# mmeidlinger/lut_ldpc

Measured on AMD Instinct MI355X. Metric: decoded codewords/sec, DVB-S2 N=64800 4-bit LUT 50-iter, higher is better.
Workload: dtype u8

## Files before the change

### lut_ldpc_amd/csrc/hip/decoder_frontend.hip

```cpp
#include "decoder_state.hpp"
#include "kernels_frontend.hpp"
#include "kernels_encode.hpp"

#pragma GCC visibility push(hidden)

hipError_t preload_frontend_kernels() {
    hipFuncAttributes a;
    return hipFuncGetAttributes(&a, reinterpret_cast<const void *>(&encode_random_kernel));
}

static int fill_cells(const lutldpc_channel_cells *c, const lutldpc_decoder *d, ChannelCells &C) {
    if (!c || !c->thr || !c->cha_label || !c->msg_label || !c->slicer_neg || !c->cha_label_mirror || !c->msg_label_mirror)
        return fail(LUTLDPC_ERR_ARG, "channel cells: NULL member");
    if (c->n_cells < 1 || c->n_cells > kMaxCells) return fail(LUTLDPC_ERR_ARG, "channel cells: n_cells outside [1,72]");
    std::memset(&C, 0, sizeof(C));
    C.n_cells = c->n_cells;
    for (int j = 0; j < c->n_cells; j++) {
        if (j < c->n_cells - 1) { C.thr[j] = c->thr[j]; if (j && c->thr[j] < c->thr[j - 1]) return fail(LUTLDPC_ERR_ARG, "channel cells: thresholds must ascend"); }
        if (c->cha_label[j] >= d->Nq_Cha || c->cha_label_mirror[j] >= d->Nq_Cha || c->msg_label[j] >= d->Nq_Msg[0] || c->msg_label_mirror[j] >= d->Nq_Msg[0])
            return fail(LUTLDPC_ERR_ARG, "channel cells: label outside its alphabet");
        C.cha[j] = c->cha_label[j]; C.msg[j] = c->msg_label[j]; C.neg[j] = c->slicer_neg[j] ? 1 : 0;
        C.cha_m[j] = c->cha_label_mirror[j]; C.msg_m[j] = c->msg_label_mirror[j];
    }
    return LUTLDPC_OK;
// ... 8 lines not shown
    HIP_TRY(hipMemsetAsync(d->d_stats.p, 0, sizeof(int32_t) * (size_t)Bpad * 4, d->stream));
    const uint8_t *cw = nullptr;
    if (codewords_host) {
        HIP_TRY(d->d_codewords.alloc((size_t)B * N));
        HIP_TRY(hipMemcpyAsync(d->d_codewords.p, codewords_host, (size_t)B * N, hipMemcpyHostToDevice, d->stream));
        cw = d->d_codewords.p;
    }
    Timed t(d, LUTLDPC_K_FRONTEND);
    const int ppt = 8, npairs = (N + 1) / 2;
    dim3 grid((unsigned)((npairs + 4 * ppt - 1) / (4 * ppt)), (unsigned)G);
    DEV_PARAM(dC, d, C);
    if (sent_rows)
        PACK_DISPATCH(d, launch_k(sample_labels_kernel<PK, true>, grid, dim3(256), 0, d->stream, dC, (uint32_t)seed, (uint32_t)(seed >> 32), stream, frame0, B, N,
                           sent_rows, d->d_cha_t.p, d->d_msg0_t.p, d->d_stats.p, ppt));
    else
        PACK_DISPATCH(d, launch_k(sample_labels_kernel<PK>, grid, dim3(256), 0, d->stream, dC, (uint32_t)seed, (uint32_t)(seed >> 32), stream, frame0, B, N, cw,
                           d->d_cha_t.p, d->d_msg0_t.p, d->d_stats.p, ppt));
    LAUNCH_CHECK();
    return LUTLDPC_OK;
}

static int encode_tiles(lutldpc_decoder *d, uint64_t seed, uint32_t stream, uint64_t frame0, int B) {
    if (!d->gen_set) return fail(LUTLDPC_ERR_STATE, "no generator set: random codewords on the device need lutldpc_decoder_set_generator first");
    const int Bpad = d->bpad(B), G = Bpad / d->tile(), N = d->nvar;
    const int RB = d->pack == 2 ? sent_row_bytes<2>() : sent_row_bytes<1>();
    HIP_TRY(d->d_sent.alloc((size_t)G * N * RB));
    Timed t(d, LUTLDPC_K_FRONTEND);
    const int K = d->gen_K, R = d->gen_R;
    const int W128 = (K + 127) / 128, T = (R + kEncTileRows - 1) / kEncTileRows, W32 = (K + 31) / 32;
    const unsigned gx = (unsigned)(Bpad / kEncFrames), gy = (unsigned)std::max(1, (std::max(T, (W32 + 7) / 8) + 3) / 4);
    launch_k(encode_random_kernel, dim3(gx, gy), dim3(256), (size_t)W128 * kEncFrames * 16, d->stream, d->d_gen.p, K, R, d->gen_W32p,
             (uint32_t)seed, (uint32_t)(seed >> 32), stream, frame0, B, N, d->tile(), d->d_sent.p);
    LAUNCH_CHECK();
    return LUTLDPC_OK;
}

static int launch_sent_to_bytes(lutldpc_decoder *d, uint8_t *dst, int B) {
    const size_t n = (size_t)B * d->nvar;
    PACK_DISPATCH(d, launch_k(sent_rows_to_bytes_kernel<PK>, dim3((unsigned)((n + 255) / 256)), dim3(256), 0, d->stream, d->d_sent.p, B, d->nvar, dst));
    LAUNCH_CHECK();
    return LUTLDPC_OK;
}

static int sim_batch_impl(lutldpc_decoder *d, const lutldpc_channel_cells *cells, uint64_t seed, uint32_t stream, uint64_t frame0, int B,
                   const uint8_t *codewords, bool device_codewords, int K_info, int32_t *frame_stats, uint8_t *cha_out, uint8_t *bits_out) {
    if (!d || !frame_stats) return fail(LUTLDPC_ERR_ARG, "NULL argument");
    if (d->device < 0) return fail(LUTLDPC_ERR_STATE, "decoder was created without a device (host-only handle)");
    if (B <= 0 || K_info < 0 || K_info > d->nvar) return fail(LUTLDPC_ERR_ARG, "bad B / K_info");
    if (device_codewords && !d->gen_set) return fail(LUTLDPC_ERR_STATE, "sim_batch_random: no generator set (lutldpc_decoder_set_generator)");
    ChannelCells C;
    int rc = fill_cells(cells, d, C);
    if (rc) return rc;
    HIP_TRY(hipSetDevice(d->device));
    if (device_codewords) {
        if ((rc = ensure_batch(d, B))) return rc;
        if ((rc = encode_tiles(d, seed, stream, frame0, B))) return rc;
    }
    if ((rc = sample_tiles(d, C, seed, stream, frame0, B, codewords, device_codewords ? d->d_sent.p : nullptr))) return rc;
    if ((rc = decode_tiles(d, B))) return rc;
    {
        Timed t(d, LUTLDPC_K_FRONTEND);
        const int Bpad = d->bpad(B), G = Bpad / d->tile(), rpw = 64;
        const int rows = K_info > 0 ? K_info : 1;
        const dim3 grid((unsigned)((rows + 4 * rpw - 1) / (4 * rpw)), (unsigned)G);
        if (device_codewords)
            PACK_DISPATCH(d, launch_k(count_errors_kernel<PK, true>, grid, dim3(256), 0, d->stream, d->d_hard.p, d->d_sent.p, B, d->nvar, K_info, d->d_iters.p,
                               d->d_stats.p, rpw));
        else
            PACK_DISPATCH(d, launch_k(count_errors_kernel<PK>, grid, dim3(256), 0, d->stream, d->d_hard.p,
                               codewords ? d->d_codewords.p : nullptr, B, d->nvar, K_info, d->d_iters.p, d->d_stats.p, rpw));
        LAUNCH_CHECK();
    }
    HIP_TRY(hipMemcpyAsync(frame_stats, d->d_stats.p, sizeof(int32_t) * (size_t)B * 4, hipMemcpyDeviceToHost, d->stream));
    if (cha_out || bits_out) {
        const int Bpad = d->bpad(B), G = Bpad / d->tile(), N = d->nvar;
        const size_t n = (size_t)B * N;
        HIP_TRY(d->d_out_bits.alloc(n));
        if (cha_out) {
            if ((rc = launch_transpose_out(d, d->d_cha_t.p, d->d_out_bits.p, B, G))) return rc;
            LAUNCH_CHECK();
            HIP_TRY(hipMemcpyAsync(cha_out, d->d_out_bits.p, n, hipMemcpyDeviceToHost, d->stream));
        }
        if (bits_out) {
            if ((rc = launch_transpose_out(d, d->d_hard.p, d->d_out_bits.p, B, G))) return rc;
            LAUNCH_CHECK();
            HIP_TRY(hipMemcpyAsync(bits_out, d->d_out_bits.p, n, hipMemcpyDeviceToHost, d->stream));
        }
    }
    HIP_TRY(hipStreamSynchronize(d->stream));
    return LUTLDPC_OK;
}

#pragma GCC visibility pop

extern "C" {

int lutldpc_decoder_sim_batch(lutldpc_decoder *d, const lutldpc_channel_cells *cells, uint64_t seed, uint32_t stream, uint64_t frame0, int B,
                              const uint8_t *codewords, int K_info, int32_t *frame_stats, uint8_t *cha_out, uint8_t *bits_out) {
    return sim_batch_impl(d, cells, seed, stream, frame0, B, codewords, false, K_info, frame_stats, cha_out, bits_out);
}

int lutldpc_decoder_sim_batch_random(lutldpc_decoder *d, const lutldpc_channel_cells *cells, uint64_t seed, uint32_t stream, uint64_t frame0, int B,
                                     int K_info, int32_t *frame_stats, uint8_t *cha_out, uint8_t *bits_out) {
    return sim_batch_impl(d, cells, seed, stream, frame0, B, nullptr, true, K_info, frame_stats, cha_out, bits_out);
}

int lutldpc_decoder_set_generator(lutldpc_decoder *d, int K, int R, const uint64_t *rows) {
    if (!d) return fail(LUTLDPC_ERR_ARG, "NULL decoder");
    if (!rows) return fail(LUTLDPC_ERR_ARG, "generator rows are NULL");
    if (K < 1 || R < 0 || K + R != d->nvar) return fail(LUTLDPC_ERR_ARG, "generator: K + R must equal nvar (K >= 1)");
    if (d->device < 0) return fail(LUTLDPC_ERR_STATE, "decoder was created without a device (host-only handle)");
    if (K > kEncMaxInfoBits) return fail(LUTLDPC_ERR_UNSUPPORTED, "generator: more than 8192 information bits (device encoder limit)");
    HIP_TRY(hipSetDevice(d->device));
    const int WK = (K + 63) / 64, W32p = 4 * ((K + 127) / 128), Rp = (R + kEncTileRows - 1) / kEncTileRows * kEncTileRows;
    std::vector<uint32_t> a((size_t)std::max(Rp, 1) * W32p, 0u);
    for (int i = 0; i < R; i++)
        for (int j = 0; j < 2 * WK; j++) {
            const int k0 = 32 * j;
            uint32_t w = (uint32_t)(rows[(size_t)i * WK + (size_t)(j >> 1)] >> (32 * (j & 1)));
            if (k0 + 32 > K) w &= k0 >= K ? 0u : (1u << (K - k0)) - 1u;
            a[(size_t)i * W32p + (size_t)j] = w;
        }
    HIP_TRY(hipStreamSynchronize(d->stream));
    HIP_TRY(d->d_gen.upload(a));
    d->gen_K = K; d->gen_R = R; d->gen_W32p = W32p; d->gen_set = true;
    make_describe(d);
    return LUTLDPC_OK;
}

int lutldpc_decoder_encode_random(lutldpc_decoder *d, uint64_t seed, uint32_t stream, uint64_t frame0, int B, uint8_t *codewords) {
    if (!d) return fail(LUTLDPC_ERR_ARG, "NULL decoder");
    if (B <= 0) return fail(LUTLDPC_ERR_ARG, "B must be positive");
    if (d->device < 0) return fail(LUTLDPC_ERR_STATE, "decoder was created without a device (host-only handle)");
    HIP_TRY(hipSetDevice(d->device));
    int rc = encode_tiles(d, seed, stream, frame0, B);
    if (rc) return rc;
    if (codewords) {
        const size_t n = (size_t)B * d->nvar;
        HIP_TRY(d->d_out_bits.alloc(n));
        if ((rc = launch_sent_to_bytes(d, d->d_out_bits.p, B))) return rc;
        HIP_TRY(hipMemcpyAsync(codewords, d->d_out_bits.p, n, hipMemcpyDeviceToHost, d->stream));
    }
    HIP_TRY(hipStreamSynchronize(d->stream));
    return LUTLDPC_OK;
}

int lutldpc_decoder_sample_labels(lutldpc_decoder *d, const lutldpc_channel_cells *cells, uint64_t seed, uint32_t stream, uint64_t frame0, int B,
                                  const uint8_t *codewords, uint8_t *cha, uint8_t *msg0) {
    if (!d || !cha || !msg0) return fail(LUTLDPC_ERR_ARG, "NULL argument");
    if (d->device < 0) return fail(LUTLDPC_ERR_STATE, "decoder was created without a device (host-only handle)");
    if (B <= 0) return fail(LUTLDPC_ERR_ARG, "B must be positive");
    ChannelCells C;
    int rc = fill_cells(cells, d, C);
    if (rc) return rc;
    HIP_TRY(hipSetDevice(d->device));
    if ((rc = sample_tiles(d, C, seed, stream, frame0, B, codewords))) return rc;
    const int Bpad = d->bpad(B), G = Bpad / d->tile(), N = d->nvar;
    const size_t n = (size_t)B * N;
    HIP_TRY(d->d_in_cha.alloc(n)); HIP_TRY(d->d_in_msg.alloc(n));
    if ((rc = launch_transpose_out(d, d->d_cha_t.p, d->d_in_cha.p, B, G))) return rc;
    if ((rc = launch_transpose_out(d, d->d_msg0_t.p, d->d_in_msg.p, B, G))) return rc;
    HIP_TRY(hipMemcpyAsync(cha, d->d_in_cha.p, n, hipMemcpyDeviceToHost, d->stream));
    HIP_TRY(hipMemcpyAsync(msg0, d->d_in_msg.p, n, hipMemcpyDeviceToHost, d->stream));
    HIP_TRY(hipStreamSynchronize(d->stream));
    return LUTLDPC_OK;
}

// ... 2 lines not shown
```

### lut_ldpc_amd/csrc/hip/decoder_state.hpp

```cpp
#pragma once
#include "../../../include/lut_ldpc_hip.h"
#include "kernels_common.hpp"
#include "kernels_fast.hpp"
#include "lut_program.hpp"
#include "jit.hpp"
#include "jit_resident.hpp"

#include <algorithm>
#include <array>
#include <cmath>
#include <cstdio>
#include <cstring>
#include <map>
#include <memory>
#include <mutex>
#include <sstream>
#include <string>
#include <vector>

namespace lutldpc { LUTLDPC_FAST_LAUNCHERS(extern) }

using namespace lutldpc;

#pragma GCC visibility push(hidden)
// ... 159 lines not shown
    std::vector<std::vector<const JitKernel *>> var_jit, dec_jit, chk_jit;
    std::string jit_log;
    struct GraphSlot { int seen = 0; hipGraphExec_t exec = nullptr; };
    std::map<std::array<int, 4>, GraphSlot> graphs;
    void drop_graphs() { for (auto &kv : graphs) if (kv.second.exec) (void)hipGraphExecDestroy(kv.second.exec); graphs.clear(); }
    int cn_epw() const { return opt.cn_edges_per_wave > 0 ? opt.cn_edges_per_wave : 42; }
    int npw_vn(int deg) const { return opt.nodes_per_wave > 0 ? opt.nodes_per_wave : std::max(1, opt.vn_edges_per_wave / std::max(deg, 1)); }
    int npw_cn(int deg) const { return opt.nodes_per_wave_cn > 0 ? opt.nodes_per_wave_cn : std::max(1, cn_epw() / std::max(deg, 1)); }
    int npw_cn_class(size_t ci) const { return ci < cn_npw_class.size() && cn_npw_class[ci] > 0 ? cn_npw_class[ci] : npw_cn(cclass[ci].deg); }
    std::string place_info = "null";
    struct SkewSlot { int n_roles = 0; size_t role_off = 0; const int32_t *items = nullptr; int nb = 0; int state_half = -1, state_ii = 0; };
    struct SkewPlan { std::vector<SkewSlot> slots; std::vector<RoleParams> h_roles; DevBuf<RoleParams> d_roles; };
    std::map<std::array<int, 3>, std::unique_ptr<SkewPlan>> skew_plans;
    std::map<std::pair<std::vector<int>, std::vector<int>>, DevBuf<int32_t>> item_tabs;
    void drop_plans() { skew_plans.clear(); item_tabs.clear(); }
    int tile() const { return kRowBytes * pack; }
    int bpad(int B) const { return (B + tile() - 1) / tile() * tile(); }
    bool profiling = false;
    struct Ev { hipEvent_t a, b; int kind; };
    std::vector<Ev> ev_live;
    std::vector<hipEvent_t> ev_pool;
    double prof_ms[LUTLDPC_K_COUNT] = {0};
    int64_t prof_n[LUTLDPC_K_COUNT] = {0};
    std::string describe;

    lutldpc_decoder() = default;
    lutldpc_decoder(const lutldpc_decoder &) = delete;
    lutldpc_decoder &operator=(const lutldpc_decoder &) = delete;
    ~lutldpc_decoder();
};

#pragma GCC visibility push(hidden)

#define LAUNCH_CHECK()                                                                              \
    do {                                                                                            \
        hipError_t e_ = hipGetLastError();                                                          \
        if (e_ != hipSuccess) return fail(LUTLDPC_ERR_HIP, std::string("kernel launch: ") + hipGetErrorString(e_)); \
        if (d->opt.validate) {                                                                      \
            e_ = hipStreamSynchronize(d->stream);                                                   \
            if (e_ == hipSuccess) e_ = hipGetLastError();                                           \
            if (e_ != hipSuccess) return fail(LUTLDPC_ERR_HIP, std::string("launch failed on the device (") + __func__ + ":" + std::to_string(__LINE__) + "): " + hipGetErrorString(e_)); \
        }                                                                                           \
    } while (0)

const void *dev_param_bytes(lutldpc_decoder *d, const void *src, size_t n);
template <class T> const T *dev_param(lutldpc_decoder *d, const T &v) { return static_cast<const T *>(dev_param_bytes(d, &v, sizeof(T))); }
#define DEV_PARAM(var, d, v)                      \
    const auto *var = dev_param((d), (v));        \
    if (!var) return LUTLDPC_ERR_HIP

#define PACK_DISPATCH(d, ...)                        \
    do {                                             \
        if ((d)->pack == 2) { constexpr int PK = 2; __VA_ARGS__; } \
        else { constexpr int PK = 1; __VA_ARGS__; }  \
    } while (0)

hipEvent_t ev_get(lutldpc_decoder *d);
void prof_fold(lutldpc_decoder *d);
struct Timed {
    lutldpc_decoder *d; int kind; hipEvent_t a{}, b{};
    Timed(lutldpc_decoder *d_, int k) : d(d_), kind(k) {
        if (d->profiling) { a = ev_get(d); b = ev_get(d); (void)hipEventRecord(a, d->stream); }
    }
    ~Timed() {
        if (d->profiling) { (void)hipEventRecord(b, d->stream); d->ev_live.push_back({a, b, kind}); }
    }
};
void make_describe(lutldpc_decoder *d);

void build_classes(const std::vector<int> &deg, std::vector<NodeClass> &cls, std::vector<int> &list);
int compile_all(lutldpc_decoder *d);
int upload_static(lutldpc_decoder *d);
struct JitRegistry { std::mutex mu; std::map<std::string, JitKernel> by_src; };
constexpr size_t kJitRegistryMax = 4096;
JitRegistry &jit_registry();
JitKernel *jit_get(int device, const std::string &src, std::string &log);
bool jit_class_source(const lutldpc_decoder *d, int kind, size_t s, size_t i, std::string &src, std::string &err);

int ensure_batch(lutldpc_decoder *d, int B);
int check_batch_buffers(const lutldpc_decoder *d, int Bpad);

hipError_t preload_stream_kernels();
int launch_state(lutldpc_decoder *d, int B, int Bpad, int mode, int value, int f0 = 0, int f1 = -1, int sel = 0);
int launch_transpose_out(lutldpc_decoder *d, const uint8_t *src_rows, uint8_t *dst, int B, int G, int rows = 0);
int launch_quantize_llr(lutldpc_decoder *d, size_t n, int n_qb_Cha, int n_qb_Msg, int mode);
bool chain_active(const lutldpc_decoder *d, int set);
bool late_hard_active(const lutldpc_decoder *d, bool skewed, bool *chain_skip);
int launch_late_hard(lutldpc_decoder *d, bool skewed, int g0, int G, const int32_t *ctl);
int decode_tiles(lutldpc_decoder *d, int B);
int decode_device(lutldpc_decoder *d, const uint8_t *d_cha, const uint8_t *d_msg0, int B, uint8_t *d_out_bits, int32_t *d_out_iters);

struct HalfRange { int g0, G; };
hipError_t preload_compact_kernels();
bool skew_eligible(const lutldpc_decoder *d);
bool compaction_on(const lutldpc_decoder *d, int G);
int compaction_min_groups(const lutldpc_decoder *d);
int launch_uncompaction(lutldpc_decoder *d, const HalfRange (&half)[2], int Bpad);
int iterate_skewed(lutldpc_decoder *d, int B, int Bpad, int G);

ResidentSpec resident_spec(const lutldpc_decoder *d, int S, int NT);
bool resident_eligible(const lutldpc_decoder *d);
bool resident_pick(const lutldpc_decoder *d, int G, int &S_out, int &NT_out, int &lds_out);
inline bool resident_active(const lutldpc_decoder *d) { return d->resident_ok && d->opt.use_resident; }
int resident_plan_for(lutldpc_decoder *d, int G, lutldpc_decoder::ResidentPlan **out);
int launch_resident(lutldpc_decoder *d, int G, int B);

hipError_t preload_frontend_kernels();

#pragma GCC visibility pop
```

### lut_ldpc_amd/csrc/hip/decoder_stream.hip

```cpp
#include "decoder_state.hpp"
#include "kernels_generic.hpp"

#pragma GCC visibility push(hidden)

hipError_t preload_stream_kernels() {
    hipFuncAttributes a;
    return hipFuncGetAttributes(&a, reinterpret_cast<const void *>(&frame_state_kernel));
}

int launch_state(lutldpc_decoder *d, int B, int Bpad, int mode, int value, int f0, int f1, int sel) {
    Timed t(d, LUTLDPC_K_LAYOUT);
    if (f1 < 0) f1 = Bpad;
    if (f1 <= f0) return LUTLDPC_OK;
    if (mode == 0) HIP_TRY(hipMemsetAsync(d->d_vfail.p + (size_t)kVfailSlots * d->Bcap, 0, (size_t)kVfailSlots * d->Bcap, d->stream));
    launch_k(frame_state_kernel, dim3((unsigned)((f1 - f0) / 256)), dim3(256), 0, d->stream,
                       d->d_state.p, d->d_vfail.p + (size_t)sel * kVfailSlots * d->Bcap, d->d_iters.p, B, f0, f1, mode, value, d->Bcap);
    LAUNCH_CHECK();
    return LUTLDPC_OK;
}

static int launch_syndrome(lutldpc_decoder *d, int G, int sel = 0) {
    Timed t(d, LUTLDPC_K_SYNDROME);
    const int cpw = 8;
    unsigned bx = (unsigned)((d->nchk + 4 * cpw - 1) / (4 * cpw));
    PACK_DISPATCH(d, launch_k(syndrome_bits_kernel<PK>, dim3(bx, (unsigned)G), dim3(256), 0, d->stream, d->d_hard.p,
                       reinterpret_cast<const uint32_t *>(d->d_state.p), reinterpret_cast<uint32_t *>(d->d_vfail.p + (size_t)sel * kVfailSlots * d->Bcap),
                       d->d_cn_ptr.p, reinterpret_cast<const uint32_t *>(d->d_cn_vn.p), d->nchk, d->nvar, cpw, d->Bcap / 4, -1, (const int32_t *)nullptr, (int32_t *)nullptr));
    LAUNCH_CHECK();
    return LUTLDPC_OK;
}
static int launch_syndrome_of_labels(lutldpc_decoder *d, int G) {
    Timed t(d, LUTLDPC_K_SYNDROME);
    const int cpw = 8, sbit = __builtin_ctz((unsigned)(d->Nq_Cha / 2));
    HIP_TRY(hipMemsetAsync(d->d_grp.p, 0, sizeof(int32_t) * (size_t)G, d->stream));
#define SYN_ARGS(CPW, SKIP, OUT) d->d_cha_t.p, reinterpret_cast<const uint32_t *>(d->d_state.p), reinterpret_cast<uint32_t *>(d->d_vfail.p), d->d_cn_ptr.p, \
                     reinterpret_cast<const uint32_t *>(d->d_cn_vn.p), d->nchk, d->nvar, CPW, d->Bcap / 4, sbit, SKIP, OUT
    PACK_DISPATCH(d, launch_k(syndrome_bits_kernel<PK>, dim3(1u, (unsigned)G), dim3(64), 0, d->stream, SYN_ARGS(64, (const int32_t *)nullptr, d->d_grp.p)));
    unsigned bx = (unsigned)((d->nchk + 4 * cpw - 1) / (4 * cpw));
    PACK_DISPATCH(d, launch_k(syndrome_bits_kernel<PK>, dim3(bx, (unsigned)G), dim3(256), 0, d->stream, SYN_ARGS(cpw, (const int32_t *)d->d_grp.p, (int32_t *)nullptr)));
#undef SYN_ARGS
    LAUNCH_CHECK();
    return LUTLDPC_OK;
}

static int launch_transpose_in(lutldpc_decoder *d, const uint8_t *src, uint8_t *dst_rows, int B, int G, int limit) {
    const int N = d->nvar;
    if (N % 4 == 0 && (reinterpret_cast<uintptr_t>(src) & 3u) == 0)
        PACK_DISPATCH(d, launch_k(transpose_in_vec_kernel<PK>, dim3((unsigned)((N + 127) / 128), (unsigned)G), dim3(256), 0, d->stream, src, dst_rows, B, N, limit));
    else
        PACK_DISPATCH(d, launch_k(transpose_in_kernel<PK>, dim3((unsigned)((N + 31) / 32), (unsigned)G), dim3(256), 0, d->stream, src, dst_rows, B, N, limit));
    LAUNCH_CHECK();
    return LUTLDPC_OK;
}
int launch_transpose_out(lutldpc_decoder *d, const uint8_t *src_rows, uint8_t *dst, int B, int G, int rows) {
    const int N = rows > 0 ? rows : d->nvar;
    if (N % 4 == 0 && (reinterpret_cast<uintptr_t>(dst) & 3u) == 0)
        PACK_DISPATCH(d, launch_k(transpose_out_vec_kernel<PK>, dim3((unsigned)((N + 127) / 128), (unsigned)G), dim3(256), 0, d->stream, src_rows, dst, B, N));
    else
        PACK_DISPATCH(d, launch_k(transpose_out_kernel<PK>, dim3((unsigned)((N + 31) / 32), (unsigned)G), dim3(256), 0, d->stream, src_rows, dst, B, N));
    LAUNCH_CHECK();
    return LUTLDPC_OK;
}

static PassParams filter_params(const PassParams &P, const std::vector<char> &keep) {
    PassParams Q = P;
    Q.n_seg = 0;
    int blk = 0;
    for (int i = 0; i < P.n_seg; i++) {
        if (!keep[(size_t)i]) continue;
        PassSeg S = P.seg[i];
        S.block_begin = blk;
        blk += (S.n_nodes + P.nodes_per_block - 1) / P.nodes_per_block;
        Q.seg[Q.n_seg++] = S;
    }
    Q.blocks_per_group = blk;
    return Q;
}

template <int KIND>
static int launch_tree_pass(lutldpc_decoder *d, PassPlan &plan, std::vector<FastClassPlan> *fast, const std::vector<const JitKernel *> *jit, int G, int nz, int check, int write_hard, int kind_id,
                     const std::vector<std::pair<int, int>> *jit_tabs = nullptr) {
    if (!plan.valid) return fail(LUTLDPC_ERR_STATE, "pass plan missing for this tree set");
    Timed t(d, kind_id);
    PassParams P = plan.P;
    P.G = G; P.nz = nz; P.check = check; P.write_hard = write_hard; P.vfail_stride_w = d->Bcap / 4;
    std::vector<char> keep((size_t)P.n_seg, 1);
    bool any = false;
    const bool sign_bit = KIND != TT_VAR || is_pow2(nz);
    if (d->opt.use_fast && fast && KIND != TT_CHK && sign_bit)
        for (int i = 0; i < P.n_seg; i++) {
            if (!(*fast)[(size_t)i].ok) continue;
            bool ok = false;
            FastParams FP = (*fast)[(size_t)i].P;
            fill_vn_fast(FP, G, nz, check, write_hard, d->npw_vn(FP.deg), d->E, d->nvar, d->Bcap / 4);
            DEV_PARAM(dFP, d, FP);
            PACK_DISPATCH(d, ok = launch_vn_fast<KIND, PK>(d->stream, FP, dFP, d->d_msgs.p, d->d_cha_t.p, d->d_hard.p,
                                     reinterpret_cast<const uint32_t *>(d->d_state.p), reinterpret_cast<uint32_t *>(d->d_vfail.p), d->d_tables.p, d->d_fast_idx.p));
            if (ok) keep[(size_t)i] = 0;
        }
    if (jit && sign_bit)
        for (int i = 0; i < P.n_seg && (size_t)i < jit->size(); i++) {
            const JitKernel *k = (*jit)[(size_t)i];
            if (!keep[(size_t)i] || !k) continue;
            FastParams F{};
            F.n_nodes = P.seg[i].n_nodes; F.deg = P.seg[i].deg;
            F.idx_off = KIND == TT_CHK ? d->cn_idx_off[(size_t)i] : d->vn_idx_off[(size_t)i];
            F.nodes_per_wave = KIND == TT_CHK ? d->npw_cn(F.deg) : d->npw_vn(F.deg); F.waves_per_group = (F.n_nodes + F.nodes_per_wave - 1) / F.nodes_per_wave;
            F.G = G; F.E = d->E; F.N = d->nvar; F.g0 = 0; F.nz = nz; F.check = check; F.write_hard = write_hard; F.vfail_stride_w = d->Bcap / 4;
            F.tab_off[0] = P.seg[i].tab_off; F.tab_len[0] = P.seg[i].tab_bytes;
            if (jit_tabs && (size_t)i < jit_tabs->size() && (*jit_tabs)[(size_t)i].second > 0) { F.tab_off[0] = (*jit_tabs)[(size_t)i].first; F.tab_len[0] = (*jit_tabs)[(size_t)i].second; }
            uint8_t *msgs = d->d_msgs.p, *hard = d->d_hard.p;
            const uint8_t *cha = d->d_cha_t.p, *tables = d->d_tables.p;
            const uint32_t *state_w = reinterpret_cast<const uint32_t *>(d->d_state.p);
            uint32_t *vfail_w = reinterpret_cast<uint32_t *>(d->d_vfail.p);
            const int32_t *fidx = d->d_fast_idx.p;
            DEV_PARAM(dF, d, F);
            void *args[] = {&dF, &msgs, &cha, &hard, &state_w, &vfail_w, &tables, &fidx};
            const unsigned blocks = (unsigned)((F.waves_per_group * G + 3) / 4);
            HIP_TRY(hipModuleLaunchKernel(k->fn, blocks, 1, 1, 256, 1, 1, 0, d->stream, args, nullptr));
            keep[(size_t)i] = 0;
        }
    for (char k : keep) any = any || k;
    if (any) {
        P = filter_params(P, keep);
        DEV_PARAM(dP, d, P);
        dim3 grid((unsigned)(P.blocks_per_group * G)), block(64);
        const int32_t *list = KIND == TT_CHK ? d->d_cn_list.p : d->d_vn_list.p;
        const int32_t *ptr = KIND == TT_CHK ? d->d_cn_ptr.p : d->d_vn_ptr.p;
        if (plan.lds_tab)
            PACK_DISPATCH(d, launch_k(tree_pass_kernel<KIND, true, PK>, grid, block, (size_t)plan.lds_bytes, d->stream, dP, d->d_msgs.p, d->d_cha_t.p,
                               d->d_hard.p, reinterpret_cast<const uint32_t *>(d->d_state.p), reinterpret_cast<uint32_t *>(d->d_vfail.p),
                               d->d_ops.p, d->d_tables.p, list, ptr, d->d_cn_idx.p, plan.out_slots));
        else
            PACK_DISPATCH(d, launch_k(tree_pass_kernel<KIND, false, PK>, grid, block, (size_t)plan.lds_bytes, d->stream, dP, d->d_msgs.p, d->d_cha_t.p,
                               d->d_hard.p, reinterpret_cast<const uint32_t *>(d->d_state.p), reinterpret_cast<uint32_t *>(d->d_vfail.p),
                               d->d_ops.p, d->d_tables.p, list, ptr, d->d_cn_idx.p, plan.out_slots));
    }
    LAUNCH_CHECK();
    return LUTLDPC_OK;
}

// ... 126 lines not shown
    if (tracing && (rc = trace_dump(d))) return rc;
    if (skewed && (rc = iterate_skewed(d, B, Bpad, G))) return rc;
    for (int ii = 0; ii < I && !skewed; ii++) {
        const int set = d->iter_set[(size_t)ii];
        const int nz_in = d->Nq_Msg[(size_t)ii] / 2;
        const int chk_check = (d->psc && ii > 0) ? 1 : 0;
        if (d->min_lut) rc = launch_cn_minsum(d, G, nz_in, chk_check);
        else rc = launch_tree_pass<TT_CHK>(d, d->chk_plan[(size_t)set], nullptr, d->chk_jit.empty() ? nullptr : &d->chk_jit[(size_t)set], G, nz_in, chk_check, 0, LUTLDPC_K_CN_PASS,
                                           (size_t)set < d->chk_full_tab.size() ? &d->chk_full_tab[(size_t)set] : nullptr);
        if (rc) return rc;
        if (chk_check && (rc = launch_state(d, B, Bpad, 2, ii))) return rc;
        if (d->trace.level > 2 && (rc = trace_dump(d))) return rc;
        if (ii != I - 1) {
            const int nz_out = d->Nq_Msg[(size_t)(ii + 1)] / 2;
            rc = launch_tree_pass<TT_VAR>(d, d->var_plan[(size_t)set], &d->var_fast[(size_t)set], d->var_jit.empty() ? nullptr : &d->var_jit[(size_t)set], G, nz_out, d->psc ? 1 : 0,
                                          (d->psc && !late_hard_active(d, false, nullptr)) ? 1 : 0, LUTLDPC_K_VN_PASS);
            if (rc) return rc;
        }
        if (tracing && (rc = trace_dump(d))) return rc;
    }
    {
        Timed t(d, LUTLDPC_K_LAYOUT);
        if ((rc = launch_late_hard(d, skewed, 0, G, nullptr))) return rc;
        if (skewed && d->psc && d->pisc && compaction_on(d, G) && late_hard_active(d, true, nullptr) && d->opt.compact_keep) {
            PACK_DISPATCH(d, launch_k(hard_from_labels_masked_kernel<PK>, dim3(std::min<unsigned>(1024u, (unsigned)((N + 3) / 4)), (unsigned)G), dim3(256), 0, d->stream,
                                                d->d_cha_t.p, d->d_hard.p, reinterpret_cast<const uint32_t *>(d->d_state.p), N, d->Nq_Cha / 2, 0));
            LAUNCH_CHECK();
        }
    }
    if ((rc = launch_tree_pass<TT_DEC>(d, d->dec_plan[(size_t)last_set], &d->dec_fast[(size_t)last_set], d->dec_jit.empty() ? nullptr : &d->dec_jit[(size_t)last_set], G, 0, 0, 0, LUTLDPC_K_DECISION))) return rc;
    const int fsel = skewed ? (I & 1) : 0;
    if ((rc = launch_syndrome(d, G, fsel))) return rc;
    if ((rc = launch_state(d, B, Bpad, 3, I, 0, -1, fsel))) return rc;
    if (skewed && d->psc && compaction_on(d, G)) {
        const HalfRange half[2] = {{0, (G + 1) / 2}, {(G + 1) / 2, G - (G + 1) / 2}};
        if ((rc = launch_uncompaction(d, half, Bpad))) return rc;
    }
    if (d->profiling && d->ev_live.size() > 8192) prof_fold(d);
    return LUTLDPC_OK;
}

int decode_tiles(lutldpc_decoder *d, int B) {
    if (int rc = check_batch_buffers(d, d->bpad(B))) return rc;
    if (resident_active(d)) {
        lutldpc_decoder::ResidentPlan *pl = nullptr;
        if (int rc = resident_plan_for(d, d->bpad(B) / d->tile(), &pl)) return rc;
    }
    if (!d->opt.use_graph || d->profiling || d->trace.level > 1 || resident_active(d)) return decode_tiles_launch(d, B);
    const std::array<int, 4> key = {B, d->psc, d->pisc, d->max_iters};
    if (d->graphs.size() > 32 && !d->graphs.count(key)) d->drop_graphs();
    auto &slot = d->graphs[key];
    if (slot.exec) {
        HIP_TRY(hipGraphLaunch(slot.exec, d->stream));
        return LUTLDPC_OK;
    }
    if (slot.seen++ == 0) return decode_tiles_launch(d, B);
    HIP_TRY(hipStreamBeginCapture(d->stream, hipStreamCaptureModeThreadLocal));
    const int rc = decode_tiles_launch(d, B);
    hipGraph_t g = nullptr;
    const hipError_t e = hipStreamEndCapture(d->stream, &g);
    if (rc || e != hipSuccess || !g) {
        if (g) (void)hipGraphDestroy(g);
        (void)hipGetLastError();
        d->opt.use_graph = 0;
        return rc ? rc : decode_tiles_launch(d, B);
    }
    const hipError_t ei = hipGraphInstantiate(&slot.exec, g, nullptr, nullptr, 0);
    (void)hipGraphDestroy(g);
    if (ei != hipSuccess) { slot.exec = nullptr; d->opt.use_graph = 0; (void)hipGetLastError(); return decode_tiles_launch(d, B); }
    HIP_TRY(hipGraphLaunch(slot.exec, d->stream));
    return LUTLDPC_OK;
}

int decode_device(lutldpc_decoder *d, const uint8_t *d_cha, const uint8_t *d_msg0, int B, uint8_t *d_out_bits, int32_t *d_out_iters) {
    if (d->device < 0) return fail(LUTLDPC_ERR_STATE, "decoder was created without a device (host-only handle)");
    if (B <= 0) return fail(LUTLDPC_ERR_ARG, "B must be positive");
    HIP_TRY(hipSetDevice(d->device));
    int rc = ensure_batch(d, B);
    if (rc) return rc;
    const int Bpad = d->bpad(B), G = Bpad / d->tile();
    const bool direct = resident_active(d) && d->opt.resident_fm && d->trace.level <= 1;
    if (!direct) {
        Timed t(d, LUTLDPC_K_LAYOUT);
        if ((rc = launch_transpose_in(d, d_cha, d->d_cha_t.p, B, G, d->Nq_Cha))) return rc;
        if ((rc = launch_transpose_in(d, d_msg0, d->d_msg0_t.p, B, G, d->Nq_Msg[0]))) return rc;
        LAUNCH_CHECK();
    }
    if (direct) { d->fm_cha = d_cha; d->fm_msg0 = d_msg0; d->fm_bits = d_out_bits; }
    rc = decode_tiles(d, B);
    d->fm_cha = d->fm_msg0 = nullptr; d->fm_bits = nullptr;
    if (rc) return rc;
    {
        Timed t(d, LUTLDPC_K_LAYOUT);
        if (!direct && (rc = launch_transpose_out(d, d->d_hard.p, d_out_bits, B, G))) return rc;
        HIP_TRY(hipMemcpyAsync(d_out_iters, d->d_iters.p, sizeof(int32_t) * (size_t)B, hipMemcpyDeviceToDevice, d->stream));
    }
    return LUTLDPC_OK;
}

#pragma GCC visibility pop
```

### lut_ldpc_amd/csrc/hip/kernels_generic.hpp

```cpp
#pragma once
#include "kernels_common.hpp"
#include "lut_program.hpp"

namespace lutldpc {

template <int KIND, bool LDS_TAB, int PACK>
__global__ __launch_bounds__(64) void tree_pass_kernel(
    const PassParams *__restrict__ Pp, uint8_t *__restrict__ msgs, const uint8_t *__restrict__ cha, uint8_t *__restrict__ hard,
    const uint32_t *__restrict__ state_w, uint32_t *__restrict__ vfail_w, const Op *__restrict__ ops,
    const uint8_t *__restrict__ tables, const int32_t *__restrict__ node_list,
    const int32_t *__restrict__ node_ptr,
    const int32_t *__restrict__ cn_idx, int out_slots)
{
    extern __shared__ uint32_t lds[];
    const PassParams &P = *Pp;
    const int lane = threadIdx.x;
    const int g = blockIdx.x / P.blocks_per_group;
    const int b = blockIdx.x - g * P.blocks_per_group;
    const int si = find_seg(P, b);
    const PassSeg S = P.seg[si];

    uint32_t amask[PACK];
    if (load_active<PACK>(state_w, g, lane, amask)) return;
    const uint32_t smask = pack_masks<PACK>(amask);
// ... 246 lines not shown
    const uint32_t a = __builtin_amdgcn_perm(d[1], d[0], 0x05010400u), b = __builtin_amdgcn_perm(d[1], d[0], 0x07030602u);
    const uint32_t c = __builtin_amdgcn_perm(d[3], d[2], 0x05010400u), e = __builtin_amdgcn_perm(d[3], d[2], 0x07030602u);
    d[0] = __builtin_amdgcn_perm(c, a, 0x05040100u); d[1] = __builtin_amdgcn_perm(c, a, 0x07060302u);
    d[2] = __builtin_amdgcn_perm(e, b, 0x05040100u); d[3] = __builtin_amdgcn_perm(e, b, 0x07060302u);
}

template <int PACK>
__global__ __launch_bounds__(256) void transpose_in_vec_kernel(const uint8_t *__restrict__ src, uint8_t *__restrict__ dst, int B, int N, int limit)
{
    constexpr int F = kRowBytes * PACK, FPL = 4 * PACK;
    __shared__ uint32_t tile[F * 32];
    int bx, by;
    xcd_block(bx, by);
    const int g = by, n0 = bx * 128, t = threadIdx.x;
    const int c = t & 31, fq = t >> 5;
    const uint32_t lim = (uint32_t)(limit - 1);
    for (int f0 = fq; f0 < F; f0 += 64) {
        uint32_t v[8];
#pragma unroll
        for (int j = 0; j < 8; j++) {
            const int fr = g * F + f0 + 8 * j, n = n0 + 4 * c;
            v[j] = (fr < B && n < N) ? *reinterpret_cast<const uint32_t *>(src + (size_t)fr * N + n) : 0u;
        }
#pragma unroll
        for (int j = 0; j < 8; j++) {
            const int f = f0 + 8 * j;
            const uint32_t b0 = min(v[j] & 0xFFu, lim), b1 = min((v[j] >> 8) & 0xFFu, lim), b2 = min((v[j] >> 16) & 0xFFu, lim), b3 = min(v[j] >> 24, lim);
            tile[f * 32 + (c ^ ((f / FPL) & 31))] = b0 | (b1 << 8) | (b2 << 16) | (b3 << 24);
        }
    }
    __syncthreads();
    const int lane = t & 63;
    for (int q = t >> 6; q < 32; q += 4) {
        if (n0 + 4 * q >= N) break;
        uint32_t out[4] = {0, 0, 0, 0};
#pragma unroll
        for (int h = 0; h < PACK; h++) {
            uint32_t d[4];
#pragma unroll
            for (int k = 0; k < 4; k++) d[k] = tile[(FPL * lane + 4 * h + k) * 32 + (q ^ (lane & 31))];
            transpose4x4(d);
#pragma unroll
            for (int k = 0; k < 4; k++) out[k] |= d[k] << (4 * h);
        }
#pragma unroll
        for (int k = 0; k < 4; k++)
            *reinterpret_cast<uint32_t *>(dst + ((size_t)g * N + n0 + 4 * q + k) * kRowBytes + lane * 4) = out[k];
    }
}

template <int PACK>
__global__ __launch_bounds__(256) void transpose_out_vec_kernel(const uint8_t *__restrict__ src, uint8_t *__restrict__ dst, int B, int N)
{
    constexpr int F = kRowBytes * PACK, FPL = 4 * PACK;
    __shared__ uint32_t tile[F * 32];
    int bx, by;
    xcd_block(bx, by);
    const int g = by, n0 = bx * 128, t = threadIdx.x;
    const int lane = t & 63;
    for (int q = t >> 6; q < 32; q += 4) {
        uint32_t x[4] = {0, 0, 0, 0};
        if (n0 + 4 * q < N) {
#pragma unroll
            for (int k = 0; k < 4; k++) x[k] = *reinterpret_cast<const uint32_t *>(src + ((size_t)g * N + n0 + 4 * q + k) * kRowBytes + lane * 4);
        }
#pragma unroll
        for (int h = 0; h < PACK; h++) {
            uint32_t d[4];
#pragma unroll
            for (int k = 0; k < 4; k++) d[k] = unpack_half<PACK>(x[k], h);
            transpose4x4(d);
#pragma unroll
            for (int k = 0; k < 4; k++) tile[(FPL * lane + 4 * h + k) * 32 + (q ^ (lane & 31))] = d[k];
        }
    }
    __syncthreads();
    const int c = t & 31, fq = t >> 5;
    for (int f = fq; f < F; f += 8) {
        const int fr = g * F + f, n = n0 + 4 * c;
        if (fr < B && n < N) *reinterpret_cast<uint32_t *>(dst + (size_t)fr * N + n) = tile[f * 32 + (c ^ ((f / FPL) & 31))];
    }
}

__global__ __launch_bounds__(256) void init_edges_kernel(const uint8_t *__restrict__ msg0_t, uint8_t *__restrict__ msgs,
                                                         const int32_t *__restrict__ vn_ptr, int N, int E)
{
    const int lane = threadIdx.x & 63;
    const int v = blockIdx.x * 4 + (threadIdx.x >> 6), g = blockIdx.y;
    if (v >= N) return;
    const uint32_t w = *reinterpret_cast<const uint32_t *>(msg0_t + ((size_t)g * N + v) * kRowBytes + lane * 4);
    const int e0 = vn_ptr[v], e1 = vn_ptr[v + 1];
    for (int e = e0; e < e1; e++) *reinterpret_cast<uint32_t *>(msgs + ((size_t)g * E + e) * kRowBytes + lane * 4) = w;
}

template <int PACK>
__global__ __launch_bounds__(256) void hard_from_labels_kernel(const uint8_t *__restrict__ cha_t, uint8_t *__restrict__ hard,
                                                               size_t n_words, int nz)
{
    const size_t i = (size_t)blockIdx.x * 256 + threadIdx.x;
    if (i >= n_words) return;
    const uint32_t x = reinterpret_cast<const uint32_t *>(cha_t)[i];
    uint32_t r[PACK];
#pragma unroll
    for (int h = 0; h < PACK; h++) r[h] = swar_lt(unpack_half<PACK>(x, h), (uint32_t)nz);
    reinterpret_cast<uint32_t *>(hard)[i] = pack_halves<PACK>(r);
}

template <int PACK>
__global__ __launch_bounds__(256) void hard_from_labels_masked_kernel(const uint8_t *__restrict__ cha_t, uint8_t *__restrict__ hard,
                                                                      const uint32_t *__restrict__ state_w, int N, int nz, int g0)
{
    const int lane = threadIdx.x & 63, g = g0 + blockIdx.y;
    uint32_t m[PACK], any = 0;
#pragma unroll
    for (int h = 0; h < PACK; h++) { m[h] = swar_zero_mask(state_w[frame_word<PACK>(g, lane, h)] ^ (ST_DONE_PISC * 0x01010101u)); any |= m[h]; }
    if (wave_all_zero(any)) return;
    const uint32_t smask = pack_masks<PACK>(m);
    const int w0 = __builtin_amdgcn_readfirstlane(blockIdx.x * 4 + (threadIdx.x >> 6)), step = (int)gridDim.x * 4;
    for (int v = w0; v < N; v += step) {
        const uint32_t x = *reinterpret_cast<const uint32_t *>(cha_t + ((size_t)g * N + (size_t)v) * kRowBytes + lane * 4);
        uint32_t r[PACK];
#pragma unroll
        for (int h = 0; h < PACK; h++) r[h] = swar_lt(unpack_half<PACK>(x, h), (uint32_t)nz);
        store_row_masked<PACK>(reinterpret_cast<uint32_t *>(hard + ((size_t)g * N + (size_t)v) * kRowBytes + lane * 4), pack_halves<PACK>(r), smask);
    }
}

template <int PACK>
__global__ __launch_bounds__(256) void hard_from_frozen_kernel(const uint8_t *__restrict__ msgs, uint8_t *__restrict__ hard,
                                                               const uint32_t *__restrict__ state_w, const int32_t *__restrict__ vn_ptr,
                                                               const uint8_t *__restrict__ skip, int N, int E, int nz, int g0, const int32_t *__restrict__ ctl)
{
    if (ctl && ctl[1]) return;
    const int lane = threadIdx.x & 63, g = g0 + blockIdx.y;
    uint32_t m[PACK], any = 0;
#pragma unroll
    for (int h = 0; h < PACK; h++) { m[h] = swar_zero_mask(state_w[frame_word<PACK>(g, lane, h)] ^ (ST_DONE_PSC * 0x01010101u)); any |= m[h]; }
    if (wave_all_zero(any)) return;
    const uint32_t smask = pack_masks<PACK>(m);
    const int w0 = __builtin_amdgcn_readfirstlane(blockIdx.x * 4 + (threadIdx.x >> 6)), step = (int)gridDim.x * 4;
#pragma unroll 4
    for (int v = w0; v < N; v += step) {
        if (skip && skip[v]) continue;
        const uint32_t x = *reinterpret_cast<const uint32_t *>(msgs + ((size_t)g * E + (size_t)vn_ptr[v]) * kRowBytes + lane * 4);
        uint32_t r[PACK];
#pragma unroll
        for (int h = 0; h < PACK; h++) r[h] = swar_lt(unpack_half<PACK>(x, h), (uint32_t)nz);
        store_row_masked<PACK>(reinterpret_cast<uint32_t *>(hard + ((size_t)g * N + (size_t)v) * kRowBytes + lane * 4), pack_halves<PACK>(r), smask);
    }
}

template <int PACK>
__global__ __launch_bounds__(256) void chain_hard_kernel(uint8_t *__restrict__ hard, const uint32_t *__restrict__ state_w, const int32_t *__restrict__ edges,
                                                         const int32_t *__restrict__ links, const int32_t *__restrict__ edge_vn, int n_nodes, int deg, int npw, int N,
                                                         int g0, const int32_t *__restrict__ ctl)
{
    if (ctl && ctl[1]) return;
    const int lane = threadIdx.x & 63, g = g0 + blockIdx.y;
    uint32_t m[PACK], any = 0;
#pragma unroll
    for (int h = 0; h < PACK; h++) { m[h] = swar_zero_mask(state_w[frame_word<PACK>(g, lane, h)] ^ (ST_DONE_PSC * 0x01010101u)); any |= m[h]; }
    if (wave_all_zero(any)) return;
    const uint32_t smask = pack_masks<PACK>(m);
    const int runs = (n_nodes + npw - 1) / npw;
    const int w0 = __builtin_amdgcn_readfirstlane(blockIdx.x * 4 + (threadIdx.x >> 6)), step = (int)gridDim.x * 4;
    uint8_t *hb = hard + (size_t)g * (size_t)N * kRowBytes + lane * 4;
// ... 100 lines not shown
```

Measured before the change: 257,200.

## Fuse input transposes into one nibble-packing kernel and add bit-only output transpose

Replaces the two separate input transpose launches (channel labels and initial messages) with a single launch using blockIdx.z to select the stream, packing two frames per byte as nibbles when PACK==2. Adds a specialized output transpose for hard bits that extracts only the low bit per frame, packs four variables into a nibble in LDS, and expands it back to bytes with a multiply. The aim is to reduce launch count and LDS/register traffic in the layout stages around decoding. It adds new specialized kernels whose index math must match the existing packed layout.

Result: no change. 256,600 (-0.2%).

```diff
diff --git a/lut_ldpc_amd/csrc/hip/decoder_frontend.hip b/lut_ldpc_amd/csrc/hip/decoder_frontend.hip
--- a/lut_ldpc_amd/csrc/hip/decoder_frontend.hip
+++ b/lut_ldpc_amd/csrc/hip/decoder_frontend.hip
@@ -114,7 +114,7 @@
             HIP_TRY(hipMemcpyAsync(cha_out, d->d_out_bits.p, n, hipMemcpyDeviceToHost, d->stream));
         }
         if (bits_out) {
-            if ((rc = launch_transpose_out(d, d->d_hard.p, d->d_out_bits.p, B, G))) return rc;
+            if ((rc = launch_transpose_out(d, d->d_hard.p, d->d_out_bits.p, B, G, 0, true))) return rc;
             LAUNCH_CHECK();
             HIP_TRY(hipMemcpyAsync(bits_out, d->d_out_bits.p, n, hipMemcpyDeviceToHost, d->stream));
         }
diff --git a/lut_ldpc_amd/csrc/hip/decoder_state.hpp b/lut_ldpc_amd/csrc/hip/decoder_state.hpp
--- a/lut_ldpc_amd/csrc/hip/decoder_state.hpp
+++ b/lut_ldpc_amd/csrc/hip/decoder_state.hpp
@@ -265,7 +265,7 @@
 
 hipError_t preload_stream_kernels();
 int launch_state(lutldpc_decoder *d, int B, int Bpad, int mode, int value, int f0 = 0, int f1 = -1, int sel = 0);
-int launch_transpose_out(lutldpc_decoder *d, const uint8_t *src_rows, uint8_t *dst, int B, int G, int rows = 0);
+int launch_transpose_out(lutldpc_decoder *d, const uint8_t *src_rows, uint8_t *dst, int B, int G, int rows = 0, bool bits = false);
 int launch_quantize_llr(lutldpc_decoder *d, size_t n, int n_qb_Cha, int n_qb_Msg, int mode);
 bool chain_active(const lutldpc_decoder *d, int set);
 bool late_hard_active(const lutldpc_decoder *d, bool skewed, bool *chain_skip);
diff --git a/lut_ldpc_amd/csrc/hip/decoder_stream.hip b/lut_ldpc_amd/csrc/hip/decoder_stream.hip
--- a/lut_ldpc_amd/csrc/hip/decoder_stream.hip
+++ b/lut_ldpc_amd/csrc/hip/decoder_stream.hip
@@ -43,20 +43,29 @@
     return LUTLDPC_OK;
 }
 
-static int launch_transpose_in(lutldpc_decoder *d, const uint8_t *src, uint8_t *dst_rows, int B, int G, int limit) {
+static int launch_transpose_in(lutldpc_decoder *d, const uint8_t *const src[2], uint8_t *const dst_rows[2], const int limit[2], int B, int G) {
     const int N = d->nvar;
-    if (N % 4 == 0 && (reinterpret_cast<uintptr_t>(src) & 3u) == 0)
-        PACK_DISPATCH(d, launch_k(transpose_in_vec_kernel<PK>, dim3((unsigned)((N + 127) / 128), (unsigned)G), dim3(256), 0, d->stream, src, dst_rows, B, N, limit));
-    else
-        PACK_DISPATCH(d, launch_k(transpose_in_kernel<PK>, dim3((unsigned)((N + 31) / 32), (unsigned)G), dim3(256), 0, d->stream, src, dst_rows, B, N, limit));
-    LAUNCH_CHECK();
-    return LUTLDPC_OK;
-}
-int launch_transpose_out(lutldpc_decoder *d, const uint8_t *src_rows, uint8_t *dst, int B, int G, int rows) {
+    const bool vec = N % 4 == 0 && ((reinterpret_cast<uintptr_t>(src[0]) | reinterpret_cast<uintptr_t>(src[1])) & 3u) == 0;
+    if (vec && d->pack == 2) {
+        const TransposeInPair A = {{src[0], src[1]}, {dst_rows[0], dst_rows[1]}, {limit[0], limit[1]}};
+        launch_k(transpose_in_nib_kernel, dim3((unsigned)((N + 127) / 128), (unsigned)G, 2u), dim3(256), 0, d->stream, A, B, N);
+    } else
+        for (int z = 0; z < 2; z++) {
+            if (vec)
+                PACK_DISPATCH(d, launch_k(transpose_in_vec_kernel<PK>, dim3((unsigned)((N + 127) / 128), (unsigned)G), dim3(256), 0, d->stream, src[z], dst_rows[z], B, N, limit[z]));
+            else
+                PACK_DISPATCH(d, launch_k(transpose_in_kernel<PK>, dim3((unsigned)((N + 31) / 32), (unsigned)G), dim3(256), 0, d->stream, src[z], dst_rows[z], B, N, limit[z]));
+        }
+    LAUNCH_CHECK();
+    return LUTLDPC_OK;
+}
+int launch_transpose_out(lutldpc_decoder *d, const uint8_t *src_rows, uint8_t *dst, int B, int G, int rows, bool bits) {
     const int N = rows > 0 ? rows : d->nvar;
-    if (N % 4 == 0 && (reinterpret_cast<uintptr_t>(dst) & 3u) == 0)
-        PACK_DISPATCH(d, launch_k(transpose_out_vec_kernel<PK>, dim3((unsigned)((N + 127) / 128), (unsigned)G), dim3(256), 0, d->stream, src_rows, dst, B, N));
-    else
+    const dim3 grid((unsigned)((N + 127) / 128), (unsigned)G);
+    if (N % 4 == 0 && (reinterpret_cast<uintptr_t>(dst) & 3u) == 0) {
+        if (bits) PACK_DISPATCH(d, launch_k(transpose_out_bits_kernel<PK>, grid, dim3(256), 0, d->stream, src_rows, dst, B, N));
+        else PACK_DISPATCH(d, launch_k(transpose_out_vec_kernel<PK>, grid, dim3(256), 0, d->stream, src_rows, dst, B, N));
+    } else
         PACK_DISPATCH(d, launch_k(transpose_out_kernel<PK>, dim3((unsigned)((N + 31) / 32), (unsigned)G), dim3(256), 0, d->stream, src_rows, dst, B, N));
     LAUNCH_CHECK();
     return LUTLDPC_OK;
@@ -349,9 +358,10 @@
     const bool direct = resident_active(d) && d->opt.resident_fm && d->trace.level <= 1;
     if (!direct) {
         Timed t(d, LUTLDPC_K_LAYOUT);
-        if ((rc = launch_transpose_in(d, d_cha, d->d_cha_t.p, B, G, d->Nq_Cha))) return rc;
-        if ((rc = launch_transpose_in(d, d_msg0, d->d_msg0_t.p, B, G, d->Nq_Msg[0]))) return rc;
-        LAUNCH_CHECK();
+        const uint8_t *const src[2] = {d_cha, d_msg0};
+        uint8_t *const rows[2] = {d->d_cha_t.p, d->d_msg0_t.p};
+        const int limit[2] = {d->Nq_Cha, d->Nq_Msg[0]};
+        if ((rc = launch_transpose_in(d, src, rows, limit, B, G))) return rc;
     }
     if (direct) { d->fm_cha = d_cha; d->fm_msg0 = d_msg0; d->fm_bits = d_out_bits; }
     rc = decode_tiles(d, B);
@@ -359,7 +369,7 @@
     if (rc) return rc;
     {
         Timed t(d, LUTLDPC_K_LAYOUT);
-        if (!direct && (rc = launch_transpose_out(d, d->d_hard.p, d_out_bits, B, G))) return rc;
+        if (!direct && (rc = launch_transpose_out(d, d->d_hard.p, d_out_bits, B, G, 0, true))) return rc;
         HIP_TRY(hipMemcpyAsync(d_out_iters, d->d_iters.p, sizeof(int32_t) * (size_t)B, hipMemcpyDeviceToDevice, d->stream));
     }
     return LUTLDPC_OK;
diff --git a/lut_ldpc_amd/csrc/hip/kernels_generic.hpp b/lut_ldpc_amd/csrc/hip/kernels_generic.hpp
--- a/lut_ldpc_amd/csrc/hip/kernels_generic.hpp
+++ b/lut_ldpc_amd/csrc/hip/kernels_generic.hpp
@@ -352,6 +352,97 @@
     }
 }
 
+struct TransposeInPair {
+    const uint8_t *src[2];
+    uint8_t *dst[2];
+    int32_t limit[2];
+};
+__device__ __forceinline__ uint32_t clamp_labels(uint32_t v, uint32_t lim) {
+    return min(v & 0xFFu, lim) | (min((v >> 8) & 0xFFu, lim) << 8) | (min((v >> 16) & 0xFFu, lim) << 16) | (min(v >> 24, lim) << 24);
+}
+__global__ __launch_bounds__(256) void transpose_in_nib_kernel(TransposeInPair A, int B, int N)
+{
+    constexpr int F = kRowBytes * 2, P = F / 2;
+    __shared__ uint32_t tile[P * 32];
+    int bx, by;
+    xcd_block(bx, by);
+    const int z = blockIdx.z;
+    const uint8_t *__restrict__ src = A.src[z];
+    uint8_t *__restrict__ dst = A.dst[z];
+    const uint32_t lim = (uint32_t)(A.limit[z] - 1);
+    const int g = by, n0 = bx * 128, t = threadIdx.x;
+    const int c = t & 31, pq = t >> 5;
+    const int n = n0 + 4 * c;
+    for (int p0 = pq; p0 < P; p0 += 64) {
+        uint32_t lo[8], hi[8];
+#pragma unroll
+        for (int j = 0; j < 8; j++) {
+            const int p = p0 + 8 * j;
+            const int fr = g * F + (p >> 2) * 8 + (p & 3);
+            lo[j] = (fr < B && n < N) ? *reinterpret_cast<const uint32_t *>(src + (size_t)fr * N + n) : 0u;
+            hi[j] = (fr + 4 < B && n < N) ? *reinterpret_cast<const uint32_t *>(src + (size_t)(fr + 4) * N + n) : 0u;
+        }
+#pragma unroll
+        for (int j = 0; j < 8; j++) {
+            const int p = p0 + 8 * j;
+            tile[p * 32 + (c ^ ((p >> 2) & 31))] = clamp_labels(lo[j], lim) | (clamp_labels(hi[j], lim) << 4);
+        }
+    }
+    __syncthreads();
+    const int lane = t & 63;
+    for (int q = t >> 6; q < 32; q += 4) {
+        if (n0 + 4 * q >= N) break;
+        uint32_t d[4];
+#pragma unroll
+        for (int k = 0; k < 4; k++) d[k] = tile[(4 * lane + k) * 32 + (q ^ (lane & 31))];
+        transpose4x4(d);
+#pragma unroll
+        for (int k = 0; k < 4; k++)
+            *reinterpret_cast<uint32_t *>(dst + ((size_t)g * N + n0 + 4 * q + k) * kRowBytes + lane * 4) = d[k];
+    }
+}
+
+template <int PACK>
+__global__ __launch_bounds__(256) void transpose_out_bits_kernel(const uint8_t *__restrict__ src, uint8_t *__restrict__ dst, int B, int N)
+{
+    constexpr int F = kRowBytes * PACK, FPL = 4 * PACK;
+    constexpr uint32_t ONES = PACK == 2 ? 0x11111111u : 0x01010101u;
+    __shared__ uint32_t tile[kWave * 32];
+    int bx, by;
+    xcd_block(bx, by);
+    const int g = by, n0 = bx * 128, t = threadIdx.x;
+    const int lane = t & 63, w = t >> 6;
+#pragma unroll
+    for (int i = 0; i < 2; i++) {
+        uint32_t x[4][4];
+#pragma unroll
+        for (int j = 0; j < 4; j++) {
+            const int q = w + 4 * (4 * i + j);
+#pragma unroll
+            for (int k = 0; k < 4; k++)
+                x[j][k] = (n0 + 4 * q + k < N) ? *reinterpret_cast<const uint32_t *>(src + ((size_t)g * N + n0 + 4 * q + k) * kRowBytes + lane * 4) : 0u;
+        }
+#pragma unroll
+        for (int j = 0; j < 4; j++) {
+            const int q = w + 4 * (4 * i + j);
+            tile[lane * 32 + (q ^ (lane & 31))] = (x[j][0] & ONES) | ((x[j][1] & ONES) << 1) | ((x[j][2] & ONES) << 2) | ((x[j][3] & ONES) << 3);
+        }
+    }
+    __syncthreads();
+    const int c = t & 31, r = t >> 5;
+    const int n = n0 + 4 * c;
+    if (n >= N) return;
+    if (PACK == 1 && r >= FPL) return;
+    const int sh = PACK == 2 ? 8 * (r & 3) + 4 * (r >> 2) : 8 * r;
+#pragma unroll 8
+    for (int L = 0; L < kWave; L++) {
+        const int fr = g * F + L * FPL + r;
+        if (fr >= B) break;
+        const uint32_t nib = (tile[L * 32 + (c ^ (L & 31))] >> sh) & 0xFu;
+        *reinterpret_cast<uint32_t *>(dst + (size_t)fr * N + n) = (nib * 0x00204081u) & 0x01010101u;
+    }
+}
+
 __global__ __launch_bounds__(256) void init_edges_kernel(const uint8_t *__restrict__ msg0_t, uint8_t *__restrict__ msgs,
                                                          const int32_t *__restrict__ vn_ptr, int N, int E)
 {
```
